# codelion/adaptive-classifier

Measured on AMD Instinct MI355X. Metric: predict() queries/sec + kNN GB/s vs HBM roofline, 768-d, higher is better.
Workload: dtype f32

## Files before the change

### adaptive-classifier_amd/adaptive_classifier/_native.py

```python
import ctypes
import os
import subprocess

import torch

_HERE = os.path.dirname(os.path.abspath(__file__))
_LIB_PATH = os.environ.get("AC_LIBACAMD_PATH") or os.path.join(_HERE, "libacamd.so")
_CSRC = os.path.join(os.path.dirname(_HERE), "csrc")
_lib = None

c_void_p, c_int, c_int64, c_size_t, c_float, c_uint64 = (
    ctypes.c_void_p, ctypes.c_int, ctypes.c_int64, ctypes.c_size_t, ctypes.c_float, ctypes.c_uint64)


class NativeError(RuntimeError):
    pass


AC_GEMM_F32, AC_GEMM_BF16X3, AC_GEMM_F16X2 = 0, 1, 2
AC_BERT_LAYERED = 1
AC_BERT_PATH_PACKED, AC_BERT_PATH_PADDED, AC_BERT_PATH_PADDED_MASK = 0, 1, 2


def build(force=False):
# ... 34 lines not shown

class ac_wordpiece_vocab(ctypes.Structure):
    _fields_ = [("keys", c_void_p), ("offs", c_void_p), ("ids", c_void_p), ("lens", c_void_p), ("blob", c_void_p),
                ("slots", c_int), ("max_piece_bytes", c_int), ("unk_id", c_int), ("cls_id", c_int), ("sep_id", c_int),
                ("pad_id", c_int), ("lower_case", c_int)]


class ac_bert_weights(ctypes.Structure):
    _fields_ = [(n, c_void_p) for n in (
        "word_emb", "pos_emb", "type_emb", "emb_ln_g", "emb_ln_b",
        "qkv_w", "qkv_b", "ao_w", "ao_b", "ln1_g", "ln1_b",
        "ff1_w", "ff1_b", "ff2_w", "ff2_b", "ln2_g", "ln2_b",
        "qkv_w3", "ao_w3", "ff1_w3", "ff2_w3", "qkv_wh", "ao_wh", "ff1_wh", "ff2_wh")]


_SIGNATURES = {
    "ac_last_error": (ctypes.c_char_p, []),
    "ac_version": (c_int, []),
    "ac_device_info": (c_int, [ctypes.POINTER(c_int), ctypes.POINTER(c_int), ctypes.POINTER(c_size_t)]),
    "ac_device_cus": (c_int, [ctypes.POINTER(c_int), ctypes.POINTER(c_int)]),
    "ac_persistent_launches": (c_int, [ctypes.POINTER(c_int64), ctypes.POINTER(c_int64)]),
    "ac_knn_l2_topk_workspace": (c_int, [c_int64, c_int, c_int, c_int, ctypes.POINTER(c_size_t)]),
    "ac_knn_l2_topk": (c_int, [c_void_p, c_int64, c_int64, c_int, c_void_p, c_int, c_int64, c_int, c_int64,
                               c_void_p, c_void_p, c_void_p, c_size_t, c_void_p, c_void_p]),
    "ac_knn_l2_topk_x": (c_int, [c_void_p, c_int64, c_int64, c_int, c_void_p, c_int, c_int64, c_int, c_int64,
                                 c_void_p, c_void_p, c_void_p, c_void_p, c_size_t, c_void_p, c_void_p]),
    "ac_knn_ip_topk_workspace": (c_int, [c_int64, c_int, c_int, c_int, ctypes.POINTER(c_size_t)]),
    "ac_knn_ip_topk": (c_int, [c_void_p, c_int64, c_int64, c_int, c_void_p, c_int, c_int64, c_int, c_int64,
                               c_void_p, c_void_p, c_void_p, c_size_t, c_void_p, c_void_p]),
    "ac_knn_ip_topk_x": (c_int, [c_void_p, c_int64, c_int64, c_int, c_void_p, c_int, c_int64, c_int, c_int64,
                                 c_void_p, c_void_p, c_void_p, c_void_p, c_size_t, c_void_p, c_void_p]),
    "ac_topk_merge_ip_f64": (c_int, [c_void_p, c_void_p, c_int, c_int, c_int, c_void_p, c_void_p, c_void_p]),
    "ac_knn_store_bytes": (c_int, [c_int64, c_int, ctypes.POINTER(c_size_t), ctypes.POINTER(c_size_t)]),
    "ac_knn_prepare_store": (c_int, [c_void_p, c_int64, c_int64, c_int, c_void_p, c_void_p, c_void_p]),
    "ac_knn_update_store": (c_int, [c_void_p, c_int64, c_int64, c_int64, c_int, c_void_p, c_void_p, c_int64, c_int64, c_void_p, c_void_p]),
    "ac_knn_l2_topk_batch_workspace": (c_int, [c_int64, c_int, c_int, c_int, ctypes.POINTER(c_size_t)]),
    "ac_knn_l2_topk_batch": (c_int, [c_void_p, c_int64, c_int64, c_int, c_void_p, c_void_p, c_void_p, c_int, c_int64, c_int,
                                     c_int64, c_void_p, c_void_p, c_void_p, c_void_p, c_size_t, c_void_p, c_void_p]),
    "ac_knn_ip_topk_batch_workspace": (c_int, [c_int64, c_int, c_int, c_int, ctypes.POINTER(c_size_t)]),
    "ac_knn_ip_topk_batch": (c_int, [c_void_p, c_int64, c_int64, c_int, c_void_p, c_void_p, c_void_p, c_int, c_int64, c_int,
                                     c_int64, c_void_p, c_void_p, c_void_p, c_void_p, c_size_t, c_void_p, c_void_p]),
    "ac_knn_range_workspace": (c_int, [c_int64, c_int, c_int, ctypes.POINTER(c_size_t)]),
    "ac_knn_l2_range_count": (c_int, [c_void_p, c_int64, c_int64, c_int, c_void_p, c_int, c_int64, c_void_p, c_void_p,
                                      c_void_p, c_size_t, c_void_p, c_void_p]),
    "ac_knn_l2_range_fill": (c_int, [c_void_p, c_int64, c_int64, c_int, c_void_p, c_int, c_int64, c_int64, c_void_p, c_int64,
                                     c_void_p, c_void_p, c_void_p, c_void_p, c_size_t, c_void_p, c_void_p]),
    "ac_knn_ip_range_count": (c_int, [c_void_p, c_int64, c_int64, c_int, c_void_p, c_int, c_int64, c_void_p, c_void_p,
                                      c_void_p, c_size_t, c_void_p, c_void_p]),
    "ac_knn_ip_range_fill": (c_int, [c_void_p, c_int64, c_int64, c_int, c_void_p, c_int, c_int64, c_int64, c_void_p, c_int64,
                                     c_void_p, c_void_p, c_void_p, c_void_p, c_size_t, c_void_p, c_void_p]),
    "ac_knn_l2_topk_sel": (c_int, [c_void_p, c_int64, c_int64, c_int, c_void_p, c_int, c_int64, c_int, c_int64, c_void_p, c_int64,
                                   c_void_p, c_void_p, c_void_p, c_void_p, c_size_t, c_void_p, c_void_p]),
    "ac_knn_ip_topk_sel": (c_int, [c_void_p, c_int64, c_int64, c_int, c_void_p, c_int, c_int64, c_int, c_int64, c_void_p, c_int64,
                                   c_void_p, c_void_p, c_void_p, c_void_p, c_size_t, c_void_p, c_void_p]),
    "ac_knn_l2_topk_batch_sel": (c_int, [c_void_p, c_int64, c_int64, c_int, c_void_p, c_void_p, c_void_p, c_int, c_int64, c_int,
                                         c_int64, c_void_p, c_int64, c_void_p, c_void_p, c_void_p, c_void_p, c_size_t, c_void_p, c_void_p]),
    "ac_knn_ip_topk_batch_sel": (c_int, [c_void_p, c_int64, c_int64, c_int, c_void_p, c_void_p, c_void_p, c_int, c_int64, c_int,
                                         c_int64, c_void_p, c_int64, c_void_p, c_void_p, c_void_p, c_void_p, c_size_t, c_void_p, c_void_p]),
    "ac_knn_l2_topk_ids": (c_int, [c_void_p, c_int64, c_int64, c_int, c_void_p, c_int64, c_void_p, c_int, c_int64, c_int, c_int64,
                                   c_void_p, c_void_p, c_void_p, c_void_p]),
    "ac_knn_ip_topk_ids": (c_int, [c_void_p, c_int64, c_int64, c_int, c_void_p, c_int64, c_void_p, c_int, c_int64, c_int, c_int64,
                                   c_void_p, c_void_p, c_void_p, c_void_p]),
    "ac_knn_sel_pack": (c_int, [c_void_p, c_int64, c_void_p, c_void_p]),
    "ac_knn_sel_classes": (c_int, [c_void_p, c_int64, c_void_p, c_int, c_void_p, c_void_p]),
    "ac_knn_set_profile_events": (c_int, [c_void_p, c_void_p]),
    "ac_topk_merge": (c_int, [c_void_p, c_void_p, c_int, c_int, c_int, c_void_p, c_void_p, c_void_p]),
    "ac_topk_merge_f64": (c_int, [c_void_p, c_void_p, c_int, c_int, c_int, c_void_p, c_void_p, c_void_p]),
    "ac_rows_to_class": (c_int, [c_void_p, c_int64, c_void_p, c_int64, c_void_p, c_int, c_void_p, c_void_p]),
    "ac_proto_scores": (c_int, [c_void_p, c_void_p, c_int, c_int, c_void_p, c_void_p]),
    "ac_synth_unit_rows": (c_int, [c_void_p, c_int64, c_int64, c_int, c_uint64, c_int64, c_void_p]),
    "ac_linear_f32": (c_int, [c_void_p, c_int64, c_void_p, c_int64, c_void_p, c_void_p, c_int64, c_void_p,
                              c_int64, c_int, c_int, c_int, c_int, c_void_p]),
    "ac_gemm_f32": (c_int, [c_int, c_int, c_int, c_int, c_int, c_float, c_void_p, c_int64, c_void_p, c_int64,
                            c_float, c_void_p, c_int64, c_void_p]),
    "ac_gemm_set_arith": (c_int, [c_int]),
    "ac_gemm_get_arith": (c_int, []),
    "ac_gemm_set_variant": (c_int, [c_int]),
    "ac_gemm_debug_stamps": (c_int, [c_void_p, c_int64]),
    "ac_gemm_set_pipe_table": (c_int, [ctypes.c_char_p]),
    "ac_gemm_set_pipe_table_f16": (c_int, [ctypes.c_char_p]),
    "ac_gemm_set_krot": (c_int, [c_int]),
    "ac_gemm_set_ln_fusion": (c_int, [c_int]),
    "ac_gemm_ln_fusion_launches": (c_int64, []),
    "ac_gemm_qkv_attn_launches": (c_int64, []),
    "ac_set_persistent_kernels": (c_int, [c_int]),
    "ac_clock_stamp": (c_int, [c_void_p, c_void_p]),
    "ac_gemm_occupancy": (c_int, [c_int, c_int, ctypes.POINTER(c_int)]),
    "ac_split_bf16x3": (c_int, [c_void_p, c_int64, c_int64, c_int, c_void_p, c_void_p]),
    "ac_split_f16x2": (c_int, [c_void_p, c_int64, c_int64, c_int, c_int, c_void_p, c_void_p]),
    "ac_linear_f16x2": (c_int, [c_void_p, c_void_p, c_void_p, c_void_p, c_int64, c_void_p, c_int64, c_void_p, c_int, c_int,
                                c_int, c_int, c_void_p]),
    "ac_linear_bf16x3": (c_int, [c_void_p, c_int64, c_void_p, c_void_p, c_int64, c_void_p, c_void_p, c_void_p,
                                 c_int64, c_void_p, c_int64, c_void_p, c_int, c_int, c_int, c_int, c_void_p]),
    "ac_head_param_count": (c_int64, [ctypes.POINTER(ac_head_dims)]),
    "ac_head_workspace": (c_int, [ctypes.POINTER(ac_head_dims), c_int, ctypes.POINTER(c_size_t)]),
    "ac_head_forward": (c_int, [ctypes.POINTER(ac_head_dims), c_void_p, c_void_p, c_int64, c_int, c_void_p,
                                c_void_p, c_size_t, c_void_p]),
    "ac_head_fwd_bwd_ce": (c_int, [ctypes.POINTER(ac_head_dims), c_void_p, c_void_p, c_int64, c_void_p,
                                   c_void_p, c_void_p, c_float, c_int, c_void_p, c_void_p, c_void_p, c_size_t,
                                   c_void_p]),
    "ac_head_fwd_bwd_loss": (c_int, [ctypes.POINTER(ac_head_dims), c_void_p, c_void_p, c_int64, c_void_p, c_void_p,
                                     c_int64, c_int, c_void_p, c_void_p, c_float, c_int, c_void_p, c_void_p, c_void_p,
                                     c_size_t, c_void_p]),
    "ac_strategic_workspace": (c_int, [ctypes.POINTER(ac_head_dims), c_int, c_int, ctypes.POINTER(c_size_t)]),
    "ac_strategic_best_response": (c_int, [ctypes.POINTER(ac_head_dims), c_void_p, c_void_p, c_int64, c_int, c_void_p,
                                           c_void_p, c_int, c_void_p, c_int, c_int, c_void_p, c_void_p, c_float, c_uint64,
                                           c_void_p, c_void_p, c_void_p, c_void_p, c_int64, c_void_p, c_void_p, c_size_t,
                                           c_void_p]),
    "ac_head_fwd_bwd_strategic": (c_int, [ctypes.POINTER(ac_head_dims), c_void_p, c_void_p, c_int64, c_void_p, c_void_p,
                                          c_void_p, c_float, c_int, c_uint64, c_int, c_float, c_void_p, c_void_p, c_void_p,
                                          c_void_p, c_size_t, c_void_p]),
    "ac_sigmoid": (c_int, [c_void_p, c_int64, c_void_p, c_void_p]),
    "ac_head_train_step": (c_int, [ctypes.POINTER(ac_head_dims), c_void_p, c_void_p, c_void_p, c_void_p, c_void_p,
                                   c_int64, c_void_p, c_void_p, c_int64, c_int, c_void_p, c_int, c_float, c_uint64,
                                   c_void_p, c_void_p,
                                   c_float, c_float, c_float, c_float, c_float, c_float, c_float, c_int, c_void_p,
                                   c_void_p, c_void_p, c_size_t, c_void_p]),
    "ac_head_train_epoch": (c_int, [ctypes.POINTER(ac_head_dims), c_void_p, c_void_p, c_void_p, c_void_p, c_void_p,
                                    c_int64, c_void_p, c_void_p, c_int64, c_int, c_void_p, c_int64, c_int, c_float,
                                    c_uint64, c_void_p, c_void_p,
                                    c_float, c_float, c_float, c_float, c_float, c_float, c_float, c_int, c_void_p,
                                    c_void_p, c_void_p, c_size_t, ctypes.POINTER(c_int), c_void_p]),
    "ac_softmax_rows": (c_int, [c_void_p, c_int, c_int, c_void_p, c_void_p]),
    "ac_l2_normalize_rows": (c_int, [c_void_p, c_int64, c_int, c_int, c_void_p, c_int64, c_void_p]),
    "ac_fisher_accumulate": (c_int, [c_void_p, c_float, c_void_p, c_int64, c_void_p]),
    "ac_ewc_loss": (c_int, [c_void_p, c_void_p, c_void_p, c_int64, c_float, c_void_p, c_void_p, c_void_p]),
    "ac_ewc_adamw_step": (c_int, [c_void_p, c_void_p, c_void_p, c_void_p, c_void_p, c_void_p, c_int64, c_float,
                                  c_float, c_float, c_float, c_float, c_float, c_float, c_int, c_void_p,
                                  c_void_p, c_void_p]),
    "ac_memory_add_prune": (c_int, [c_void_p, c_void_p, c_int, c_int, c_void_p]),
    "ac_blend_topk": (c_int, [c_void_p, c_void_p, c_int, c_void_p, c_int, c_void_p, c_void_p, c_int, c_int, c_int,
                              c_void_p, c_void_p, c_void_p, c_void_p]),
    "ac_modernbert_workspace": (c_int, [ctypes.POINTER(ac_modernbert_config), c_int, c_int, ctypes.POINTER(c_size_t)]),
    "ac_modernbert_encode_cls": (c_int, [ctypes.POINTER(ac_modernbert_config), ctypes.POINTER(ac_modernbert_weights),
                                         c_void_p, c_void_p, c_int, c_int, c_void_p, c_int64, c_void_p, c_size_t,
                                         c_void_p]),
    "ac_modernbert_encode_cls_packed": (c_int, [ctypes.POINTER(ac_modernbert_config), ctypes.POINTER(ac_modernbert_weights),
                                                c_void_p, c_int, c_int, c_void_p, c_void_p, c_int, c_int, c_void_p, c_int64,
                                                c_void_p, c_size_t, c_void_p]),
    "ac_wordpiece_hash": (c_uint64, [c_void_p, c_int, c_int]),
    "ac_wordpiece_encode": (c_int, [c_void_p, c_void_p, c_int, ctypes.POINTER(ac_wordpiece_vocab), c_int, c_void_p, c_void_p,
                                    c_void_p, c_void_p]),
    "ac_bert_workspace": (c_int, [ctypes.POINTER(ac_bert_config), c_int, c_int, ctypes.POINTER(c_size_t)]),
    "ac_bert_pack": (c_int, [c_void_p, c_int, c_int, c_void_p, c_void_p, c_void_p, c_void_p]),
    "ac_bert_encode_cls_packed": (c_int, [ctypes.POINTER(ac_bert_config), ctypes.POINTER(ac_bert_weights), c_void_p, c_void_p,
                                          c_int, c_int, c_void_p, c_void_p, c_int, c_int, c_void_p, c_int64, c_void_p, c_size_t,
                                          c_void_p]),
    "ac_bert_unpad_last_wait_ns": (ctypes.c_longlong, []),
    "ac_predict_post": (c_int, [c_void_p, c_void_p, c_int, c_void_p, c_int64, c_void_p, c_int, c_void_p, c_int, c_int, c_void_p, c_void_p,
                                c_int, c_int, c_int, c_void_p, c_size_t, c_void_p, c_void_p]),
    "ac_host_alloc": (c_int, [c_size_t, ctypes.POINTER(c_void_p)]),
    "ac_host_free": (c_int, [c_void_p]),
    "ac_bert_encode_cls_unpad": (c_int, [ctypes.POINTER(ac_bert_config), ctypes.POINTER(ac_bert_weights), c_void_p, c_void_p,
                                         c_void_p, c_int, c_int, c_void_p, c_int64, c_void_p, c_size_t, c_int,
                                         ctypes.POINTER(c_int), ctypes.POINTER(c_int), c_void_p]),
    "ac_bert_encode_cls_opts": (c_int, [ctypes.POINTER(ac_bert_config), ctypes.POINTER(ac_bert_weights), c_void_p,
                                        c_void_p, c_void_p, c_int, c_int, c_void_p, c_int64, c_void_p, c_size_t, c_int,
                                        ctypes.POINTER(c_int), c_void_p]),
    "ac_bert_one_launch_status": (c_int, [ctypes.POINTER(ac_bert_config), c_int, c_int, c_void_p, c_size_t,
                                          ctypes.POINTER(c_int), c_void_p]),
    "ac_bert_ln_fusion_clear": (c_int, [c_void_p, c_size_t, c_void_p]),
    "ac_bert_ln_fusion_status": (c_int, [ctypes.POINTER(ac_bert_config), c_int, c_int, c_void_p, c_size_t,
                                         ctypes.POINTER(c_int), c_void_p]),
    "ac_bert_encode_cls": (c_int, [ctypes.POINTER(ac_bert_config), ctypes.POINTER(ac_bert_weights), c_void_p,
                                   c_void_p, c_void_p, c_int, c_int, c_void_p, c_int64, c_void_p, c_size_t,
                                   c_void_p]),
# ... 55 lines not shown
```

### adaptive-classifier_amd/csrc/gemm_pipe.hip

```cpp
#include "common.h"
#include "gemm_common.h"
#include "grid_sync.h"
#include "attention_core.h"

#include <stdio.h>
#include <stdlib.h>

#include <atomic>
#include <type_traits>

namespace {
using namespace acg;

constexpr int PSBK = 16;

struct PipeParams {
    const uint16_t* Ap; int64_t a_rows;
    const uint16_t* Wp; int64_t w_rows;
    float* C; int64_t ldc;
    int M, N, K;
    Epilogue epi;
    LnFuse ln;
    AttnFuse at;
    unsigned long long* stamps;
// ... 402 lines not shown
    wait_vm<(NS - 2) * PPW>();
    __builtin_amdgcn_sched_barrier(0);
    __builtin_amdgcn_s_barrier();
    __builtin_amdgcn_sched_barrier(0);
    stamp<(EPI == EPI_QKV_ATTN ? 16 : 4)>(prm, wave, 1);

    if constexpr (PIPE != 0) {
        Frags F0, F1;
        read_frags(F0, 0);
        int slot = 1 % NS;
        constexpr int NREAD = AR * (TM + TN), NMFMA = NPROD * TM * TN, MPR = NMFMA / NREAD;
        static_assert(MPR >= 1, "at least one MFMA per fragment read");
#define AC_PIPE_STEP(FC, FN)                                                                                     \
        do {                                                                                                     \
            wait_vm<(NS - 3) * PPW>();                         \
            __builtin_amdgcn_sched_barrier(0);                                                                   \
            __builtin_amdgcn_s_barrier();                 \
            __builtin_amdgcn_sched_barrier(0);                                                                   \
            issue();                                           \
            read_frags(FN, slot);                                                   \
            slot = slot + 1 == NS ? 0 : slot + 1;                                                                \
            mfmas(FC);                                                                               \
            if (PIPE == 2) {                              \
                _Pragma("unroll") for (int g_ = 0; g_ < NREAD; ++g_) {                                           \
                    __builtin_amdgcn_sched_group_barrier(0x008, MPR, 0);                                         \
                    __builtin_amdgcn_sched_group_barrier(0x100, 1, 0);                                           \
                }                                                                                                \
            }                                                                                                    \
        } while (0)
        for (int s = 0; s < nk; s += 2) {
            AC_PIPE_STEP(F0, F1);
            AC_PIPE_STEP(F1, F0);
        }
#undef AC_PIPE_STEP
    } else {
        int slot = 0;
        for (int s = 0; s < nk; ++s) {
            if (s > 0) {
                wait_vm<(NS - 2) * PPW>();
                __builtin_amdgcn_sched_barrier(0);
                __builtin_amdgcn_s_barrier();
                __builtin_amdgcn_sched_barrier(0);
            }
            issue();
            Frags F;
            read_frags(F, slot);
            slot = slot + 1 == NS ? 0 : slot + 1;
            mfmas(F);
        }
    }
    wait_vm<0>();
    stamp<(EPI == EPI_QKV_ATTN ? 16 : 4)>(prm, wave, 2);
    if constexpr (AR == 2) {
#pragma unroll
        for (int a = 0; a < TM; ++a)
#pragma unroll
            for (int b = 0; b < TN; ++b)
#pragma unroll
                for (int r = 0; r < 16; ++r) acc[a][b][r] *= ac::kF16OutScale;
    }
    if constexpr (EPI == EPI_BIAS_RES_LN) {
        __builtin_amdgcn_sched_barrier(0);
        __builtin_amdgcn_s_barrier();
        __builtin_amdgcn_sched_barrier(0);
        store_tile_ln<TM, TN, WMW, WNW, AR>(acc, lnres, prm, bm, bn, ntn, wm, wn, lane, tid, wave, reinterpret_cast<float*>(lds));
    } else if constexpr (EPI == EPI_QKV_ATTN) {
        __builtin_amdgcn_sched_barrier(0);
        __builtin_amdgcn_s_barrier();
        __builtin_amdgcn_sched_barrier(0);
        if constexpr (EPI == EPI_QKV_ATTN)
            qkv_attention_epilogue<TM, TN, WMW, WNW, AR>(acc, prm, bm, bn, wm, wn, lane, wave, reinterpret_cast<float*>(lds), at_cu_pref, at_bias);
    } else if (C_PLANES) {
        __builtin_amdgcn_sched_barrier(0);
        __builtin_amdgcn_s_barrier();
        __builtin_amdgcn_sched_barrier(0);
        store_tile_planes<EPI, TM, TN, AR>(acc, reinterpret_cast<uint16_t*>(prm.C), prm.M, prm.N, m0, n0, wm, wn, lane, prm.epi,
                                       reinterpret_cast<float*>(lds) + wave * kTrFloats);
    } else {
        store_tile<EPI, TM, BM, TN>(acc, prm.C, prm.ldc, prm.M, prm.N, m0, n0, wm, wn, lane, prm.epi);
    }
    if (prm.stamps) { wait_vm<0>(); stamp<(EPI == EPI_QKV_ATTN ? 16 : 4)>(prm, wave, 3); }
}

std::atomic<int> g_krot{-1};
int krot_enabled() {
    int v = g_krot.load(std::memory_order_relaxed);
    if (v < 0) {
        const char* e = getenv("AC_GEMM_KROT");
        v = (e && atoi(e) != 0) ? 1 : 0;
        g_krot.store(v, std::memory_order_relaxed);
    }
    return v;
}
unsigned long long* g_stamps = nullptr;
int64_t g_stamp_cap = 0;

template <int EPI, int TM, int TN, int WMW, int WNW, int NS, bool CP, int PIPE, int AR = 3>
int launch_one(PipeParams p, hipStream_t stream) {
    using G = PipeGeom<TM, TN, WMW, WNW, NS, AR>;
    static_assert(G::BM == 32 * TM * WMW && G::BN == 32 * TN * WNW && G::NW == WMW * WNW, "gemm_plan.h derives a ring cfg's grid and block from its digits");
    const int64_t tiles = (int64_t)((p.M + G::BM - 1) / G::BM) * ((p.N + G::BN - 1) / G::BN);
    constexpr int LN_BYTES = G::TR_BYTES + (WNW + 1) * G::BM * 8 + 16;
    const size_t lds = EPI == EPI_BIAS_RES_LN ? (size_t)(G::LDS_BYTES > LN_BYTES ? G::LDS_BYTES : LN_BYTES)
                     : EPI == EPI_QKV_ATTN    ? (size_t)(G::LDS_BYTES > kAtBytes ? G::LDS_BYTES : kAtBytes)
                                              : (size_t)(G::LDS_BYTES > G::TR_BYTES || !CP ? G::LDS_BYTES : G::TR_BYTES);
    static std::atomic<unsigned long long> attr_set{0};
    if (ac::first_call_on_device(attr_set))
        AC_HIP_CHECK(hipFuncSetAttribute((const void*)gemm_pipe_nt<EPI, TM, TN, WMW, WNW, NS, CP, PIPE, AR>,
                                         hipFuncAttributeMaxDynamicSharedMemorySize, (int)lds));
    const char* se = g_stamps ? getenv("AC_GEMM_STAMP_EPI") : nullptr;
    const char* sk = g_stamps ? getenv("AC_GEMM_STAMP_K") : nullptr;
    p.stamps = (g_stamps && tiles <= g_stamp_cap && (!se || atoi(se) == EPI) && (!sk || atoi(sk) == p.K)) ? g_stamps : nullptr;
    p.krot = krot_enabled();
    hipLaunchKernelGGL((gemm_pipe_nt<EPI, TM, TN, WMW, WNW, NS, CP, PIPE, AR>), dim3((unsigned)tiles), dim3(64 * WMW * WNW), lds, stream, p);
    AC_LAUNCH_CHECK();
    return AC_OK;
}

template <int TM, int TN, int WMW, int WNW, int NS, int PIPE, int AR = 3>
int launch_cfg(int cls, bool cp, const PipeParams& p, hipStream_t stream) {
    if (cp && cls == EPI_BIAS_GELU) return launch_one<EPI_BIAS_GELU, TM, TN, WMW, WNW, NS, true, PIPE, AR>(p, stream);
    if (cp && cls == EPI_BIAS) return launch_one<EPI_BIAS, TM, TN, WMW, WNW, NS, true, PIPE, AR>(p, stream);
    if constexpr (TN == 2 && AR == 3) if (cp && cls == EPI_GEGLU32) return launch_one<EPI_GEGLU32, TM, TN, WMW, WNW, NS, true, PIPE>(p, stream);
    if (!cp && cls == EPI_BIAS) return launch_one<EPI_BIAS, TM, TN, WMW, WNW, NS, false, PIPE, AR>(p, stream);
    if (!cp && cls == EPI_BIAS_RES) return launch_one<EPI_BIAS_RES, TM, TN, WMW, WNW, NS, false, PIPE, AR>(p, stream);
    if constexpr (TM == 1 && TN == 2 && WMW == 4 && WNW == 2 && NS == 6 && PIPE == 2)
        if (!cp && cls == EPI_BIAS_RES_LN) return launch_one<EPI_BIAS_RES_LN, TM, TN, WMW, WNW, NS, false, PIPE, AR>(p, stream);
    ac::set_error("gemm_pipe: epilogue class %d (planes out %d) not built for %s", cls, (int)cp, AR == 2 ? "fp16x2 operands" : "this tile");
    return AC_EUNSUPPORTED;
}

}

extern "C" int ac_gemm_set_krot(int on) {
    AC_TEST_HOOK_ONLY("ac_gemm_set_krot");
    g_krot.store(on ? 1 : 0, std::memory_order_relaxed);
    return AC_OK;
}
extern "C" int ac_gemm_debug_stamps(unsigned long long* d_buf, int64_t capacity_workgroups) {
    AC_TEST_HOOK_ONLY("ac_gemm_debug_stamps");
    g_stamps = d_buf;
    g_stamp_cap = d_buf ? capacity_workgroups : 0;
    return AC_OK;
}

namespace ac {

#define AC_PIPE_CONFIGS(X)                                                                         \
    X(2, 2, 2, 2, 3, 2)        \
    X(1, 2, 4, 2, 6, 1) X(1, 2, 4, 2, 6, 2)  \
    X(2, 2, 4, 2, 4, 2)                               \
    X(2, 3, 4, 2, 3, 2)                               \
    X(3, 2, 2, 4, 3, 2)                               \
    X(2, 4, 4, 2, 3, 2)

#define AC_PIPE_CONFIGS_F16(X)                                                                     \
    X(2, 4, 4, 2, 4, 2)                                           \
    X(2, 3, 4, 2, 4, 2)                                                    \
    X(2, 2, 4, 2, 6, 2)                                                    \
    X(1, 2, 4, 2, 8, 2)

int launch_gemm_pipe(int cfg, const uint16_t* Ap, int64_t a_rows, const uint16_t* Wp, int64_t w_rows, float* C, int64_t ldc,
                     uint16_t* Cp, int M, int N, int K, int cls, const acg::Epilogue& epi, hipStream_t stream, int f16) {
    PipeParams p{};
    p.Ap = Ap; p.a_rows = a_rows; p.Wp = Wp; p.w_rows = w_rows;
    p.C = Cp ? reinterpret_cast<float*>(Cp) : C; p.ldc = ldc; p.M = M; p.N = N; p.K = K; p.epi = epi;
    const bool cp = Cp != nullptr;
#define AC_CASE(TM, TN, WMW, WNW, NS, PIPE) \
    if (!f16 && cfg == (((((TM * 10 + TN) * 10 + WMW) * 10 + WNW) * 10 + NS) * 10 + PIPE)) return launch_cfg<TM, TN, WMW, WNW, NS, PIPE>(cls, cp, p, stream);
    AC_PIPE_CONFIGS(AC_CASE)
#undef AC_CASE
#define AC_CASE(TM, TN, WMW, WNW, NS, PIPE) \
    if (f16 && cfg == (((((TM * 10 + TN) * 10 + WMW) * 10 + WNW) * 10 + NS) * 10 + PIPE)) return launch_cfg<TM, TN, WMW, WNW, NS, PIPE, 2>(cls, cp, p, stream);
    AC_PIPE_CONFIGS(AC_CASE)
    AC_PIPE_CONFIGS_F16(AC_CASE)
#undef AC_CASE
    set_error("gemm_pipe: configuration %d not built", cfg);
    return AC_EUNSUPPORTED;
}


bool ln_fusion_enabled();
static int exchange_fences() {
    static const int v = [] { const char* e = getenv("AC_EXCHANGE_FENCES"); return e && atoi(e) != 0 ? 1 : 0; }();
    return v;
}
static std::atomic<long long> g_qkv_attn_launches{0};
bool qkv_attn_applies(int M, int H, int heads, int smax) {
    if (const char* e = getenv("AC_QKV_ATTN_FUSION"); e && atoi(e) == 0) return false;
    return qkv_attn_shape(M, H, heads, smax, gemm_env());
}
__global__ __launch_bounds__(kAtCu) void qkv_attn_tile_seq_kernel(const int32_t* __restrict__ cu, int b, int ntiles, int32_t* __restrict__ out) {
    const int t = blockIdx.x, i = threadIdx.x;
    auto first_at_or_after = [&](int row) { int lo = 0, hi = b; while (lo < hi) { const int mid = (lo + hi) >> 1; if (cu[mid] < row) lo = mid + 1; else hi = mid; } return lo; };
    const int sb = first_at_or_after(t * kQkvAttnRows), se = first_at_or_after((t + 1) * kQkvAttnRows), n = se - sb;
    int v = 0;
    if (i == 0) v = n;
    else if (i - 1 <= n) v = cu[sb + i - 1];
    out[(size_t)t * kAtCu + i] = v;
}
size_t qkv_attn_tile_seq_bytes(int M) { return ((size_t)(M + kQkvAttnRows - 1) / kQkvAttnRows) * kAtCu * sizeof(int32_t); }
int qkv_attn_tile_seq(const int32_t* cu, int b, int M, int32_t* tile_seq, hipStream_t stream) {
    const int ntiles = (M + kQkvAttnRows - 1) / kQkvAttnRows;
    hipLaunchKernelGGL(qkv_attn_tile_seq_kernel, dim3(ntiles), dim3(kAtCu), 0, stream, cu, b, ntiles, tile_seq);
    AC_LAUNCH_CHECK();
    return AC_OK;
}
enum { OCC_LN = 0, OCC_QKV_ATTN = 1, OCC_QKV_ATTN_F16 = 2 };
static int64_t resident_capacity(int slot, const void* fn, int threads, int lds) {
    static std::atomic<int> occ_cache[3][64];
    int dev = 0;
    if (hipGetDevice(&dev) != hipSuccess || dev < 0 || dev > 63) dev = 0;
    int occ = occ_cache[slot][dev].load(std::memory_order_relaxed);
    if (occ <= 0) {
        int per_cu = 0;
        (void)hipFuncSetAttribute(fn, hipFuncAttributeMaxDynamicSharedMemorySize, lds);
        if (hipOccupancyMaxActiveBlocksPerMultiprocessor(&per_cu, fn, threads, lds) != hipSuccess) { (void)hipGetLastError(); per_cu = 0; }
        occ = per_cu > 0 ? per_cu : -1;
        occ_cache[slot][dev].store(occ, std::memory_order_relaxed);
    }
    return occ > 0 ? (int64_t)occ * dev_info().cus : 0;
}
bool qkv_attn_exchange_applies(int M, int heads, int f16) {
    if (!ln_fusion_enabled()) return false;
    if (const char* e = getenv("AC_QKV_ATTN_EXCHANGE"); e && atoi(e) == 0) return false;
    const int64_t tiles = (int64_t)((M + kQkvAttnRows - 1) / kQkvAttnRows) * heads;
    using G16 = PipeGeom<2, 3, 4, 2, 4, 2>; using G = PipeGeom<2, 3, 4, 2, 3, 3>;
    if (f16) return tiles <= resident_capacity(OCC_QKV_ATTN_F16, (const void*)gemm_pipe_nt<EPI_QKV_ATTN, 2, 3, 4, 2, 4, false, 2, 2>, 64 * G16::NW,
                                               G16::LDS_BYTES > kAtBytes ? G16::LDS_BYTES : kAtBytes);
    return tiles <= resident_capacity(OCC_QKV_ATTN, (const void*)gemm_pipe_nt<EPI_QKV_ATTN, 2, 3, 4, 2, 3, false, 2, 3>, 64 * G::NW,
                                      G::LDS_BYTES > kAtBytes ? G::LDS_BYTES : kAtBytes);
}
int launch_gemm_pipe_qkv_attn(const uint16_t* Ap, int64_t a_rows, const uint16_t* Wp, int64_t w_rows, const float* bias, int M, int H,
                              int heads, const int32_t* cu, const int32_t* tile_seq, int b, int smax, float scale, uint16_t* ctx_planes,
                              float* qkv, hipStream_t stream, int f16, unsigned* exchange, unsigned epoch, unsigned* abort_flag) {
    AC_REQUIRE(qkv_attn_applies(M, H, heads, smax), AC_EUNSUPPORTED, "gemm_pipe: fused attention epilogue not applicable (M %d H %d heads %d longest %d)",
               M, H, heads, smax);
    AC_REQUIRE(Ap && Wp && bias && cu && tile_seq && ctx_planes && qkv && b >= 1, AC_EINVAL, "gemm_pipe_qkv_attn: null pointer");
    PipeParams p{};
    p.Ap = Ap; p.a_rows = a_rows; p.Wp = Wp; p.w_rows = w_rows; p.C = qkv; p.ldc = 3 * (int64_t)H; p.M = M; p.N = 3 * H; p.K = H;
    p.epi.bias = bias;
    p.at.cu = cu; p.at.tile_seq = tile_seq; p.at.b = b; p.at.H = H; p.at.smax = smax; p.at.scale = scale; p.at.ctx_planes = ctx_planes;
    p.at.qkv = qkv;
    AC_REQUIRE(!exchange || (abort_flag && qkv_attn_exchange_applies(M, heads, f16)), AC_EINVAL,
               "gemm_pipe_qkv_attn: the in-launch exchange needs every tile resident (%d rows x %d heads) and an abort word", M, heads);
    p.at.exchange = exchange; p.at.epoch = epoch; p.at.abort_ = abort_flag; p.at.fences = exchange_fences();
    g_qkv_attn_launches.fetch_add(1, std::memory_order_relaxed);
    return f16 ? launch_one<EPI_QKV_ATTN, 2, 3, 4, 2, 4, false, 2, 2>(p, stream)
               : launch_one<EPI_QKV_ATTN, 2, 3, 4, 2, 3, false, 2, 3>(p, stream);
}

static std::atomic<int> g_ln_fusion{-1};
static std::atomic<long long> g_ln_launches{0};
bool ln_fusion_enabled() {
    if (const int o = call_opts().ln_fusion; o >= 0) return o != 0;
    int v = g_ln_fusion.load(std::memory_order_relaxed);
    if (v < 0) {
        const char* e = getenv("AC_LN_FUSION");
        v = (e && atoi(e) == 0) ? 0 : 1;
        g_ln_fusion.store(v, std::memory_order_relaxed);
    }
    return v != 0;
}
static int64_t ln_resident_capacity() {
    using G = PipeGeom<1, 2, 4, 2, 6, 3>;
    constexpr int LN_BYTES = G::TR_BYTES + (2 + 1) * G::BM * 8 + 16;
    return resident_capacity(OCC_LN, (const void*)gemm_pipe_nt<EPI_BIAS_RES_LN, 1, 2, 4, 2, 6, false, 2, 3>, 64 * G::NW,
                             G::LDS_BYTES > LN_BYTES ? G::LDS_BYTES : LN_BYTES);
}
bool pipe_ln_applies(int M, int N, int K) {
    return ln_fusion_enabled() && pipe_ln_shape(M, N, K, gemm_env()) && tiles_of(M, N, kLnBM, kLnBN) <= ln_resident_capacity();
}
size_t pipe_ln_part_bytes(int M, int N) { return (size_t)((M + kLnBM - 1) / kLnBM) * (size_t)(N / kLnBN) * kLnBM * sizeof(float2); }
int pipe_ln_panels(int M) { return (M + kLnBM - 1) / kLnBM; }

int launch_gemm_pipe_ln(const uint16_t* Ap, int64_t a_rows, const uint16_t* Wp, int64_t w_rows, const float* bias,
                        const float* residual, int64_t ldr, float* C, int64_t ldc, int M, int N, int K, const float* gamma,
                        const float* beta, float eps, void* part, unsigned* count, unsigned* abort_flag, uint16_t* planes,
                        hipStream_t stream, int f16) {
    AC_REQUIRE(pipe_ln_applies(M, N, K), AC_EUNSUPPORTED, "gemm_pipe: fused LayerNorm epilogue not applicable to %d x %d x %d", M, N, K);
    AC_REQUIRE(Ap && Wp && bias && residual && C && gamma && beta && part && count && abort_flag, AC_EINVAL, "gemm_pipe_ln: null pointer");
    PipeParams p{};
    p.Ap = Ap; p.a_rows = a_rows; p.Wp = Wp; p.w_rows = w_rows; p.C = C; p.ldc = ldc; p.M = M; p.N = N; p.K = K;
    p.epi.bias = bias; p.epi.residual = residual; p.epi.ldr = ldr;
    p.ln.gamma = gamma; p.ln.beta = beta; p.ln.eps = eps; p.ln.part = (float2*)part; p.ln.count = count; p.ln.abort_ = abort_flag;
    p.ln.fences = exchange_fences();
    p.ln.planes = planes; p.ln.starve = (call_opts().ln_fusion >= 0 ? call_opts().ln_fusion : g_ln_fusion.load(std::memory_order_relaxed)) == 2 ? 1 : 0;
    g_ln_launches.fetch_add(1, std::memory_order_relaxed);
    return f16 ? launch_cfg<1, 2, 4, 2, 6, 2, 2>(EPI_BIAS_RES_LN, false, p, stream)
               : launch_cfg<1, 2, 4, 2, 6, 2>(EPI_BIAS_RES_LN, false, p, stream);
}
}

extern "C" int ac_gemm_set_ln_fusion(int on) {
    AC_TEST_HOOK_ONLY("ac_gemm_set_ln_fusion");
    ac::g_ln_fusion.store(on == 2 ? 2 : (on ? 1 : 0), std::memory_order_relaxed);
    return AC_OK;
}

extern "C" int64_t ac_gemm_ln_fusion_launches(void) { return (int64_t)ac::g_ln_launches.load(std::memory_order_relaxed); }
extern "C" int64_t ac_gemm_qkv_attn_launches(void) { return (int64_t)ac::g_qkv_attn_launches.load(std::memory_order_relaxed); }

static int parse_pipe_table(const char* spec, acg::PipeTable* t) {
    if (!spec) { t->n = -1; return AC_OK; }
    int n = 0;
    const char* p = spec;
    while (*p && n < 16) {
        int N = 0, K = 0, cfg = 0, used = 0;
        if (sscanf(p, "%dx%d=%d%n", &N, &K, &cfg, &used) != 3) { ac::set_error("gemm pipe table: cannot parse '%s'", p); return AC_EINVAL; }
        t->rules[n++] = {N, K, cfg};
        p += used;
        if (*p == ';') ++p;
    }
    t->n = n;
    return AC_OK;
}
extern "C" int ac_gemm_set_pipe_table(const char* spec) {
    AC_TEST_HOOK_ONLY("ac_gemm_set_pipe_table");
    return parse_pipe_table(spec, &ac::g_pipe_table);
}
extern "C" int ac_gemm_set_pipe_table_f16(const char* spec) {
    AC_TEST_HOOK_ONLY("ac_gemm_set_pipe_table_f16");
    return parse_pipe_table(spec, &ac::g_pipe_table_f16);
}
```

### include/acamd.h

```cpp
#ifndef ACAMD_H
#define ACAMD_H

#include <stddef.h>
#include <stdint.h>

#ifdef __cplusplus
extern "C" {
#endif

#define AC_OK            0
#define AC_EINVAL       -1
#define AC_EUNSUPPORTED -2
#define AC_EWORKSPACE   -3
#define AC_EHIP         -4

typedef void* ac_stream_t;

const char* ac_last_error(void);
int ac_version(void);
int ac_device_info(int* cu_count, int* lds_bytes_per_block, size_t* hbm_bytes);
int ac_device_cus(int* chip_cus, int* active_cus);
int ac_persistent_launches(int64_t* head_epoch, int64_t* bert_small);


// ... 83 lines not shown
                       float* d_outD, double* d_outD64, int64_t* d_outI,
                       void* d_ws, size_t ws_bytes, int32_t* d_stats,
                       ac_stream_t stream);
int ac_knn_ip_topk_sel(const float* d_P, int64_t N, int64_t ldP, int D,
                       const float* d_Q, int nq, int64_t ldQ, int k,
                       int64_t row_offset, const uint64_t* d_sel, int64_t sel_bit0,
                       float* d_outD, double* d_outD64, int64_t* d_outI,
                       void* d_ws, size_t ws_bytes, int32_t* d_stats,
                       ac_stream_t stream);
int ac_knn_l2_topk_batch_sel(const float* d_P, int64_t N, int64_t ldP, int D,
                             const uint16_t* d_planes, const float* d_norms,
                             const float* d_Q, int nq, int64_t ldQ, int k,
                             int64_t row_offset, const uint64_t* d_sel, int64_t sel_bit0,
                             float* d_outD, double* d_outD64, int64_t* d_outI,
                             void* d_ws, size_t ws_bytes, int32_t* d_stats,
                             ac_stream_t stream);
int ac_knn_ip_topk_batch_sel(const float* d_P, int64_t N, int64_t ldP, int D,
                             const uint16_t* d_planes, const float* d_norms,
                             const float* d_Q, int nq, int64_t ldQ, int k,
                             int64_t row_offset, const uint64_t* d_sel, int64_t sel_bit0,
                             float* d_outD, double* d_outD64, int64_t* d_outI,
                             void* d_ws, size_t ws_bytes, int32_t* d_stats,
                             ac_stream_t stream);
int ac_knn_l2_topk_ids(const float* d_P, int64_t N, int64_t ldP, int D,
                       const int64_t* d_ids, int64_t M,
                       const float* d_Q, int nq, int64_t ldQ, int k,
                       int64_t row_offset,
                       float* d_outD, double* d_outD64, int64_t* d_outI,
                       ac_stream_t stream);
int ac_knn_ip_topk_ids(const float* d_P, int64_t N, int64_t ldP, int D,
                       const int64_t* d_ids, int64_t M,
                       const float* d_Q, int nq, int64_t ldQ, int k,
                       int64_t row_offset,
                       float* d_outD, double* d_outD64, int64_t* d_outI,
                       ac_stream_t stream);
int ac_knn_sel_pack(const uint8_t* d_mask, int64_t n, uint64_t* d_sel, ac_stream_t stream);
int ac_knn_sel_classes(const int32_t* d_row_class, int64_t n, const uint8_t* d_class_on, int n_classes,
                       uint64_t* d_sel, ac_stream_t stream);

int ac_knn_set_profile_events(void* start_event, void* stop_event);

int ac_topk_merge(const float* d_D_in, const int64_t* d_I_in, int shards,
                  int nq, int k, float* d_outD, int64_t* d_outI,
                  ac_stream_t stream);
int ac_topk_merge_f64(const double* d_D_in, const int64_t* d_I_in, int shards,
                      int nq, int k, float* d_outD, int64_t* d_outI,
                      ac_stream_t stream);
int ac_topk_merge_ip_f64(const double* d_D_in, const int64_t* d_I_in, int shards,
                         int nq, int k, float* d_outD, int64_t* d_outI,
                         ac_stream_t stream);

int ac_proto_scores(const float* d_D, const int64_t* d_I, int nq, int k,
                    float* d_out, ac_stream_t stream);

int ac_rows_to_class(const int64_t* d_I, int64_t n, const int32_t* d_row_class,
                     int64_t nrows, const int64_t* d_class_lut, int nlut,
                     int64_t* d_out, ac_stream_t stream);

int ac_synth_unit_rows(float* d_out, int64_t n, int64_t ld, int D,
                       uint64_t seed, int64_t row_offset, ac_stream_t stream);


int ac_linear_f32(const float* d_A, int64_t lda, const float* d_W, int64_t ldw,
                  const float* d_bias, const float* d_residual, int64_t ldr,
                  float* d_C, int64_t ldc, int M, int N, int K, int act,
                  ac_stream_t stream);

int ac_gemm_f32(int transA, int transB, int M, int N, int K, float alpha,
                const float* d_A, int64_t lda, const float* d_B, int64_t ldb,
                float beta, float* d_C, int64_t ldc, ac_stream_t stream);

#define AC_GEMM_F32 0
#define AC_GEMM_BF16X3 1
#define AC_GEMM_F16X2 2
int ac_gemm_set_arith(int mode);
int ac_gemm_get_arith(void);
int ac_gemm_set_variant(int variant);
int ac_gemm_debug_stamps(unsigned long long* d_buf, int64_t capacity_workgroups);
int ac_gemm_set_pipe_table(const char* spec);
int ac_gemm_set_krot(int on);
int ac_gemm_set_pipe_table_f16(const char* spec);
int ac_gemm_set_ln_fusion(int on);
int64_t ac_gemm_ln_fusion_launches(void);
int64_t ac_gemm_qkv_attn_launches(void);

int ac_set_persistent_kernels(int mask);

int ac_clock_stamp(unsigned long long* d_out16, ac_stream_t stream);

int ac_gemm_occupancy(int kernel, int tm, int* blocks_per_cu);

int ac_split_bf16x3(const float* d_X, int64_t ldx, int64_t rows, int K,
                    uint16_t* d_planes, ac_stream_t stream);

int ac_split_f16x2(const float* d_X, int64_t ldx, int64_t rows, int K, int scale_log2,
                   uint16_t* d_planes, ac_stream_t stream);

int ac_linear_f16x2(const uint16_t* d_A_planes, const uint16_t* d_W_planes, const float* d_bias,
                    const float* d_residual, int64_t ldr, float* d_C, int64_t ldc, uint16_t* d_C_planes,
                    int M, int N, int K, int act, ac_stream_t stream);

int ac_linear_bf16x3(const float* d_A, int64_t lda, const uint16_t* d_A_planes,
                     const float* d_W, int64_t ldw, const uint16_t* d_W_planes,
                     const float* d_bias, const float* d_residual, int64_t ldr,
                     float* d_C, int64_t ldc, uint16_t* d_C_planes,
                     int M, int N, int K, int act, ac_stream_t stream);

typedef struct {
    int D, H1, H2, C;
} ac_head_dims;

int64_t ac_head_param_count(const ac_head_dims* dims);

int ac_head_workspace(const ac_head_dims* dims, int B, size_t* bytes);

int ac_head_forward(const ac_head_dims* dims, const float* d_params,
                    const float* d_X, int64_t ldx, int B, float* d_logits,
                    void* d_ws, size_t ws_bytes, ac_stream_t stream);

int ac_head_fwd_bwd_ce(const ac_head_dims* dims, const float* d_params,
                       const float* d_X, int64_t ldx, const int64_t* d_y,
                       const uint8_t* d_mask1, const uint8_t* d_mask2,
                       float dropout_p, int B, float* d_loss, float* d_grads,
                       void* d_ws, size_t ws_bytes, ac_stream_t stream);

#define AC_REDUCE_SCRATCH_BYTES 8192

#define AC_LOSS_CE          0
#define AC_LOSS_BCE_SIGMOID 1
#define AC_LOSS_CE_SIGMOID  2
#define AC_LOSS_STEPWISE 0x100

int ac_head_fwd_bwd_loss(const ac_head_dims* dims, const float* d_params,
                         const float* d_X, int64_t ldx, const int64_t* d_y,
                         const float* d_targets, int64_t ldt, int loss_kind,
                         const uint8_t* d_mask1, const uint8_t* d_mask2,
                         float dropout_p, int B, float* d_loss, float* d_grads,
                         void* d_ws, size_t ws_bytes, ac_stream_t stream);

int ac_sigmoid(const float* d_in, int64_t n, float* d_out, ac_stream_t stream);

int ac_head_train_step(const ac_head_dims* dims, float* d_params, float* d_m,
                       float* d_v, float* d_grads, const float* d_X, int64_t ldx,
                       const int64_t* d_y, const float* d_targets, int64_t ldt,
                       int loss_kind, const int64_t* d_index, int B,
                       float dropout_p, uint64_t dropout_seed,
                       const float* d_fisher, const float* d_old,
                       float lambda_over_B, float max_grad_norm, float lr,
                       float beta1, float beta2, float eps, float weight_decay,
                       int step, float* d_out, float* d_loss_accum,
                       void* d_ws, size_t ws_bytes, ac_stream_t stream);

int ac_head_train_epoch(const ac_head_dims* dims, float* d_params, float* d_m,
                        float* d_v, float* d_grads, const float* d_X, int64_t ldx,
                        const int64_t* d_y, const float* d_targets, int64_t ldt,
                        int loss_kind, const int64_t* d_order, int64_t n_total, int batch,
                        float dropout_p, uint64_t seed0,
                        const float* d_fisher, const float* d_old, float lambda_B,
                        float max_grad_norm, float lr, float beta1, float beta2,
                        float eps, float weight_decay, int step0,
                        float* d_out, float* d_loss_accum,
                        void* d_ws, size_t ws_bytes, int* steps_done, ac_stream_t stream);

#define AC_STRAT_COST_SEPARABLE 0
#define AC_STRAT_COST_LINEAR    1
#define AC_STRAT_MASK_NONE      0
// ... 212 lines not shown
```

Baseline: 54000.

## Add two-k-step-per-barrier pipelined GEMM kernel for fused LayerNorm epilogue

Adds a dedicated bf16x3 GEMM kernel for the bias+residual+LayerNorm fused epilogue. It processes two K-steps per workgroup barrier and double-buffers fragments, interleaving LDS fragment reads with MFMAs through sched_group_barrier. It is used by default for bf16x3 when K is a multiple of 32, and an env var can turn it off. The aim is to halve barrier and wait overhead in the K loop. In exchange, the deeper prefetch and tile residency must still fit the persistent-residency requirement of the LN exchange. The change also adds a test entry point and a launch counter.

```diff
diff --git a/adaptive-classifier_amd/adaptive_classifier/_native.py b/adaptive-classifier_amd/adaptive_classifier/_native.py
--- a/adaptive-classifier_amd/adaptive_classifier/_native.py
+++ b/adaptive-classifier_amd/adaptive_classifier/_native.py
@@ -140,6 +140,9 @@
     "ac_gemm_set_krot": (c_int, [c_int]),
     "ac_gemm_set_ln_fusion": (c_int, [c_int]),
     "ac_gemm_ln_fusion_launches": (c_int64, []),
+    "ac_gemm_ln_kstep2_launches": (c_int64, []),
+    "ac_linear_ln_bf16x3": (c_int, [c_void_p, c_void_p, c_void_p, c_void_p, c_int64, c_void_p, c_int64, c_void_p, c_int, c_int,
+                                    c_int, c_void_p, c_void_p, c_float, c_void_p, c_size_t, c_void_p]),
     "ac_gemm_qkv_attn_launches": (c_int64, []),
     "ac_set_persistent_kernels": (c_int, [c_int]),
     "ac_clock_stamp": (c_int, [c_void_p, c_void_p]),
diff --git a/adaptive-classifier_amd/csrc/gemm_pipe.hip b/adaptive-classifier_amd/csrc/gemm_pipe.hip
--- a/adaptive-classifier_amd/csrc/gemm_pipe.hip
+++ b/adaptive-classifier_amd/csrc/gemm_pipe.hip
@@ -508,6 +508,142 @@
     if (prm.stamps) { wait_vm<0>(); stamp<(EPI == EPI_QKV_ATTN ? 16 : 4)>(prm, wave, 3); }
 }
 
+__global__ __launch_bounds__(512, 2) void gemm_pipe_ln2_nt(PipeParams prm) {
+    constexpr int TM = 1, TN = 2, WMW = 4, WNW = 2, NS = 6, AR = 3;
+    using G = PipeGeom<TM, TN, WMW, WNW, NS, AR>;
+    constexpr int BM = G::BM, BN = G::BN, RA = G::RA, RG = G::RG, NP = G::NP, NW = G::NW, PPW = G::PPW, SLOT = G::SLOT;
+    static_assert(64 * NW == 512 && G::WAVES_PER_SIMD == 2, "launch bounds");
+    extern __shared__ __attribute__((aligned(16))) uint4 lds[];
+
+    const int tid = threadIdx.x, lane = tid & 63;
+    const int wave = __builtin_amdgcn_readfirstlane(tid >> 6);
+    const int wm = wave / WNW, wn = wave % WNW;
+    const int ntn = (prm.N + BN - 1) / BN;
+    const int tile = xcd_tile_id(blockIdx.x, gridDim.x);
+    const int bn = tile % ntn, bm = tile / ntn;
+    const int m0 = bm * BM, n0 = bn * BN;
+    const int nk = prm.K / PSBK;
+    stamp(prm, wave, 0);
+    float lnres[TM * TN * 16];
+    ln_prefetch_residual<TM, TN, WMW, WNW>(lnres, prm, m0, n0, wm, wn, lane);
+
+    const uint16_t* pp[PPW];
+    const int64_t a_step = 2 * prm.a_rows * 8, w_step = 2 * prm.w_rows * 8;
+    {
+        const int i32 = lane & 31, kg = lane >> 5;
+        const int64_t a_plane = prm.a_rows * (int64_t)prm.K, w_plane = prm.w_rows * (int64_t)prm.K;
+#pragma unroll
+        for (int t = 0; t < PPW; ++t) {
+            const int j = (wave + NW * t) % NP, p = j / RG, g = j % RG;
+            if (g < RA) {
+                int row = m0 + 32 * g + i32; if (row > prm.M - 1) row = prm.M - 1;
+                pp[t] = prm.Ap + p * a_plane + ((int64_t)kg * prm.a_rows + row) * 8;
+            } else {
+                int row = n0 + 32 * (g - RA) + i32; if (row > prm.N - 1) row = prm.N - 1;
+                pp[t] = prm.Wp + p * w_plane + ((int64_t)kg * prm.w_rows + row) * 8;
+            }
+        }
+    }
+    int a_cur = prm.krot ? ((int)(blockIdx.x & 7) * nk / 8) : 0;
+    if (a_cur) {
+#pragma unroll
+        for (int t = 0; t < PPW; ++t) pp[t] += (int64_t)a_cur * (((wave + NW * t) % NP) % RG < RA ? a_step : w_step);
+    }
+    const int64_t a_back = (int64_t)(nk - 1) * a_step, w_back = (int64_t)(nk - 1) * w_step;
+    int islot = 0;
+    auto issue = [&]() {
+#pragma unroll
+        for (int t = 0; t < PPW; ++t) {
+            const int j = (wave + NW * t) % NP, p = j / RG, g = j % RG;
+            __builtin_amdgcn_global_load_lds((glb_void_t*)pp[t], (lds_void_t*)&lds[islot * SLOT + (p * RG + g) * 64], 16, 0, 0);
+        }
+        const bool wrap = a_cur + 1 == nk;
+        a_cur = wrap ? 0 : a_cur + 1;
+        const int64_t da = wrap ? -a_back : a_step, dw = wrap ? -w_back : w_step;
+#pragma unroll
+        for (int t = 0; t < PPW; ++t) pp[t] += ((wave + NW * t) % NP) % RG < RA ? da : dw;
+        islot = islot + 1 == NS ? 0 : islot + 1;
+    };
+
+    f32x16 acc[TM][TN];
+#pragma unroll
+    for (int a = 0; a < TM; ++a)
+#pragma unroll
+        for (int b = 0; b < TN; ++b)
+#pragma unroll
+            for (int r = 0; r < 16; ++r) acc[a][b][r] = 0.f;
+
+    struct Frags { bf16x8_t a[TM][AR], b[TN][AR]; };
+    auto read_frags = [&](Frags& F, int slot) {
+        const uint4* base = lds + slot * SLOT + lane;
+#pragma unroll
+        for (int p = 0; p < AR; ++p) {
+#pragma unroll
+            for (int a = 0; a < TM; ++a) F.a[a][p] = __builtin_bit_cast(bf16x8_t, base[(p * RG + TM * wm + a) * 64]);
+#pragma unroll
+            for (int b = 0; b < TN; ++b) F.b[b][p] = __builtin_bit_cast(bf16x8_t, base[(p * RG + RA + TN * wn + b) * 64]);
+        }
+    };
+    auto mfmas = [&](const Frags& F) {
+        constexpr int PAIRS3[6][2] = {{2, 0}, {0, 2}, {1, 1}, {1, 0}, {0, 1}, {0, 0}};
+#pragma unroll
+        for (int pr = 0; pr < 6; ++pr)
+#pragma unroll
+            for (int a = 0; a < TM; ++a)
+#pragma unroll
+                for (int b = 0; b < TN; ++b)
+                    acc[a][b] = __builtin_amdgcn_mfma_f32_32x32x16_bf16(F.a[a][PAIRS3[pr][0]], F.b[b][PAIRS3[pr][1]], acc[a][b], 0, 0, 0);
+    };
+
+#pragma unroll
+    for (int s = 0; s < NS - 1; ++s) issue();
+    wait_vm<(NS - 2) * PPW>();
+    __builtin_amdgcn_sched_barrier(0);
+    __builtin_amdgcn_s_barrier();
+    __builtin_amdgcn_sched_barrier(0);
+    stamp(prm, wave, 1);
+
+    Frags F0, F1;
+    read_frags(F0, 0);
+    int slot = 1;
+    constexpr int NREAD = AR * (TM + TN), NMFMA = 6 * TM * TN, MPR = NMFMA / NREAD;
+    static_assert(MPR >= 1, "at least one MFMA per fragment read");
+#define AC_LN2_CHUNK(FC, FN)                                                                                     \
+    do {                                                                                                         \
+        read_frags(FN, slot);                                                    \
+        slot = slot + 1 == NS ? 0 : slot + 1;                                                                    \
+        mfmas(FC);                                                                                \
+        _Pragma("unroll") for (int g_ = 0; g_ < NREAD; ++g_) {       \
+            __builtin_amdgcn_sched_group_barrier(0x008, MPR, 0);                                                 \
+            __builtin_amdgcn_sched_group_barrier(0x100, 1, 0);                                                   \
+        }                                                                                                        \
+    } while (0)
+#define AC_LN2_STEP()                                                                                            \
+    do {                                                                                                         \
+        wait_vm<(NS - 4) * PPW>();                        \
+        asm volatile("s_waitcnt lgkmcnt(0)" ::: "memory");  \
+        __builtin_amdgcn_sched_barrier(0);                                                                       \
+        __builtin_amdgcn_s_barrier();                     \
+        __builtin_amdgcn_sched_barrier(0);                                                                       \
+        issue();                                                  \
+        AC_LN2_CHUNK(F0, F1);                                                      \
+        __builtin_amdgcn_sched_barrier(0);                                                                       \
+        issue();                                                      \
+        AC_LN2_CHUNK(F1, F0);                                                  \
+    } while (0)
+    AC_LN2_STEP();
+    for (int s = 2; s < nk; s += 2) AC_LN2_STEP();
+#undef AC_LN2_STEP
+#undef AC_LN2_CHUNK
+    wait_vm<0>();
+    stamp(prm, wave, 2);
+    __builtin_amdgcn_sched_barrier(0);
+    __builtin_amdgcn_s_barrier();
+    __builtin_amdgcn_sched_barrier(0);
+    store_tile_ln<TM, TN, WMW, WNW, AR>(acc, lnres, prm, bm, bn, ntn, wm, wn, lane, tid, wave, reinterpret_cast<float*>(lds));
+    if (prm.stamps) { wait_vm<0>(); stamp(prm, wave, 3); }
+}
+
 std::atomic<int> g_krot{-1};
 int krot_enabled() {
     int v = g_krot.load(std::memory_order_relaxed);
@@ -520,6 +656,12 @@
 }
 unsigned long long* g_stamps = nullptr;
 int64_t g_stamp_cap = 0;
+
+unsigned long long* stamp_target(int64_t tiles, int epi, int K) {
+    const char* se = g_stamps ? getenv("AC_GEMM_STAMP_EPI") : nullptr;
+    const char* sk = g_stamps ? getenv("AC_GEMM_STAMP_K") : nullptr;
+    return (g_stamps && tiles <= g_stamp_cap && (!se || atoi(se) == epi) && (!sk || atoi(sk) == K)) ? g_stamps : nullptr;
+}
 
 template <int EPI, int TM, int TN, int WMW, int WNW, int NS, bool CP, int PIPE, int AR = 3>
 int launch_one(PipeParams p, hipStream_t stream) {
@@ -534,9 +676,7 @@
     if (ac::first_call_on_device(attr_set))
         AC_HIP_CHECK(hipFuncSetAttribute((const void*)gemm_pipe_nt<EPI, TM, TN, WMW, WNW, NS, CP, PIPE, AR>,
                                          hipFuncAttributeMaxDynamicSharedMemorySize, (int)lds));
-    const char* se = g_stamps ? getenv("AC_GEMM_STAMP_EPI") : nullptr;
-    const char* sk = g_stamps ? getenv("AC_GEMM_STAMP_K") : nullptr;
-    p.stamps = (g_stamps && tiles <= g_stamp_cap && (!se || atoi(se) == EPI) && (!sk || atoi(sk) == p.K)) ? g_stamps : nullptr;
+    p.stamps = stamp_target(tiles, EPI, p.K);
     p.krot = krot_enabled();
     hipLaunchKernelGGL((gemm_pipe_nt<EPI, TM, TN, WMW, WNW, NS, CP, PIPE, AR>), dim3((unsigned)tiles), dim3(64 * WMW * WNW), lds, stream, p);
     AC_LAUNCH_CHECK();
@@ -632,9 +772,9 @@
     AC_LAUNCH_CHECK();
     return AC_OK;
 }
-enum { OCC_LN = 0, OCC_QKV_ATTN = 1, OCC_QKV_ATTN_F16 = 2 };
+enum { OCC_LN = 0, OCC_QKV_ATTN = 1, OCC_QKV_ATTN_F16 = 2, OCC_LN2 = 3, OCC_SLOTS = 4 };
 static int64_t resident_capacity(int slot, const void* fn, int threads, int lds) {
-    static std::atomic<int> occ_cache[3][64];
+    static std::atomic<int> occ_cache[OCC_SLOTS][64];
     int dev = 0;
     if (hipGetDevice(&dev) != hipSuccess || dev < 0 || dev > 63) dev = 0;
     int occ = occ_cache[slot][dev].load(std::memory_order_relaxed);
@@ -677,7 +817,7 @@
 }
 
 static std::atomic<int> g_ln_fusion{-1};
-static std::atomic<long long> g_ln_launches{0};
+static std::atomic<long long> g_ln_launches{0}, g_ln2_launches{0};
 bool ln_fusion_enabled() {
     if (const int o = call_opts().ln_fusion; o >= 0) return o != 0;
     int v = g_ln_fusion.load(std::memory_order_relaxed);
@@ -688,14 +828,22 @@
     }
     return v != 0;
 }
-static int64_t ln_resident_capacity() {
-    using G = PipeGeom<1, 2, 4, 2, 6, 3>;
-    constexpr int LN_BYTES = G::TR_BYTES + (2 + 1) * G::BM * 8 + 16;
-    return resident_capacity(OCC_LN, (const void*)gemm_pipe_nt<EPI_BIAS_RES_LN, 1, 2, 4, 2, 6, false, 2, 3>, 64 * G::NW,
-                             G::LDS_BYTES > LN_BYTES ? G::LDS_BYTES : LN_BYTES);
+static bool ln_kstep2(int K, int f16) {
+    if (f16 || (K % (2 * PSBK)) != 0) return false;
+    const char* e = getenv("AC_LN_KSTEP");
+    return !(e && atoi(e) == 1);
+}
+using LnGeom = PipeGeom<1, 2, 4, 2, 6, 3>;
+constexpr int kLnLdsBytes = LnGeom::LDS_BYTES > LnGeom::TR_BYTES + (2 + 1) * LnGeom::BM * 8 + 16 ? LnGeom::LDS_BYTES
+                                                                                                 : LnGeom::TR_BYTES + (2 + 1) * LnGeom::BM * 8 + 16;
+static int64_t ln_resident_capacity(bool kstep2) {
+    return kstep2 ? resident_capacity(OCC_LN2, (const void*)gemm_pipe_ln2_nt, 64 * LnGeom::NW, kLnLdsBytes)
+                  : resident_capacity(OCC_LN, (const void*)gemm_pipe_nt<EPI_BIAS_RES_LN, 1, 2, 4, 2, 6, false, 2, 3>, 64 * LnGeom::NW, kLnLdsBytes);
 }
 bool pipe_ln_applies(int M, int N, int K) {
-    return ln_fusion_enabled() && pipe_ln_shape(M, N, K, gemm_env()) && tiles_of(M, N, kLnBM, kLnBN) <= ln_resident_capacity();
+    if (!(ln_fusion_enabled() && pipe_ln_shape(M, N, K, gemm_env()))) return false;
+    const int64_t tiles = tiles_of(M, N, kLnBM, kLnBN);
+    return tiles <= ln_resident_capacity(false) && (!ln_kstep2(K, 0) || tiles <= ln_resident_capacity(true));
 }
 size_t pipe_ln_part_bytes(int M, int N) { return (size_t)((M + kLnBM - 1) / kLnBM) * (size_t)(N / kLnBN) * kLnBM * sizeof(float2); }
 int pipe_ln_panels(int M) { return (M + kLnBM - 1) / kLnBM; }
@@ -713,6 +861,19 @@
     p.ln.fences = exchange_fences();
     p.ln.planes = planes; p.ln.starve = (call_opts().ln_fusion >= 0 ? call_opts().ln_fusion : g_ln_fusion.load(std::memory_order_relaxed)) == 2 ? 1 : 0;
     g_ln_launches.fetch_add(1, std::memory_order_relaxed);
+    if (ln_kstep2(K, f16)) {
+        const int64_t tiles = tiles_of(M, N, kLnBM, kLnBN);
+        AC_REQUIRE(tiles <= ln_resident_capacity(true), AC_EUNSUPPORTED, "gemm_pipe_ln: %lld tiles are not resident together", (long long)tiles);
+        g_ln2_launches.fetch_add(1, std::memory_order_relaxed);
+        static std::atomic<unsigned long long> attr_set{0};
+        if (first_call_on_device(attr_set))
+            AC_HIP_CHECK(hipFuncSetAttribute((const void*)gemm_pipe_ln2_nt, hipFuncAttributeMaxDynamicSharedMemorySize, kLnLdsBytes));
+        p.stamps = stamp_target(tiles, EPI_BIAS_RES_LN, K);
+        p.krot = krot_enabled();
+        hipLaunchKernelGGL(gemm_pipe_ln2_nt, dim3((unsigned)tiles), dim3(64 * LnGeom::NW), kLnLdsBytes, stream, p);
+        AC_LAUNCH_CHECK();
+        return AC_OK;
+    }
     return f16 ? launch_cfg<1, 2, 4, 2, 6, 2, 2>(EPI_BIAS_RES_LN, false, p, stream)
                : launch_cfg<1, 2, 4, 2, 6, 2>(EPI_BIAS_RES_LN, false, p, stream);
 }
@@ -725,6 +886,20 @@
 }
 
 extern "C" int64_t ac_gemm_ln_fusion_launches(void) { return (int64_t)ac::g_ln_launches.load(std::memory_order_relaxed); }
+extern "C" int64_t ac_gemm_ln_kstep2_launches(void) { return (int64_t)ac::g_ln2_launches.load(std::memory_order_relaxed); }
+extern "C" int ac_linear_ln_bf16x3(const uint16_t* d_A_planes, const uint16_t* d_W_planes, const float* d_bias, const float* d_residual,
+                                   int64_t ldr, float* d_C, int64_t ldc, uint16_t* d_C_planes, int M, int N, int K, const float* d_gamma,
+                                   const float* d_beta, float eps, void* d_scratch, size_t scratch_bytes, ac_stream_t stream) {
+    AC_REQUIRE(M >= 1 && N >= 1 && K >= 1 && ldc >= N && ldr >= N, AC_EINVAL, "linear_ln_bf16x3: bad shape / leading dimension");
+    AC_REQUIRE(ac::pipe_ln_applies(M, N, K), AC_EUNSUPPORTED, "linear_ln_bf16x3: %d x %d x %d does not take the fused LayerNorm epilogue", M, N, K);
+    const size_t part = ac::align_up(ac::pipe_ln_part_bytes(M, N), 16), ctl = ((size_t)ac::pipe_ln_panels(M) + 1) * sizeof(unsigned);
+    AC_REQUIRE(d_scratch && scratch_bytes >= part + ctl, AC_EINVAL, "linear_ln_bf16x3: scratch of %zu bytes needed", part + ctl);
+    hipStream_t s = (hipStream_t)stream;
+    AC_HIP_CHECK(hipMemsetAsync((char*)d_scratch + part, 0, ctl, s));
+    unsigned* count = (unsigned*)((char*)d_scratch + part);
+    return ac::launch_gemm_pipe_ln(d_A_planes, M, d_W_planes, N, d_bias, d_residual, ldr, d_C, ldc, M, N, K, d_gamma, d_beta, eps, d_scratch,
+                                   count, count + ac::pipe_ln_panels(M), d_C_planes, s, 0);
+}
 extern "C" int64_t ac_gemm_qkv_attn_launches(void) { return (int64_t)ac::g_qkv_attn_launches.load(std::memory_order_relaxed); }
 
 static int parse_pipe_table(const char* spec, acg::PipeTable* t) {
diff --git a/include/acamd.h b/include/acamd.h
--- a/include/acamd.h
+++ b/include/acamd.h
@@ -189,6 +189,10 @@
 int ac_gemm_set_pipe_table_f16(const char* spec);
 int ac_gemm_set_ln_fusion(int on);
 int64_t ac_gemm_ln_fusion_launches(void);
+int64_t ac_gemm_ln_kstep2_launches(void);
+int ac_linear_ln_bf16x3(const uint16_t* d_A_planes, const uint16_t* d_W_planes, const float* d_bias, const float* d_residual,
+                        int64_t ldr, float* d_C, int64_t ldc, uint16_t* d_C_planes, int M, int N, int K, const float* d_gamma,
+                        const float* d_beta, float eps, void* d_scratch, size_t scratch_bytes, ac_stream_t stream);
 int64_t ac_gemm_qkv_attn_launches(void);
 
 int ac_set_persistent_kernels(int mask);
```

New measurement: 53920. No clear change (-0.1%).
